# jinbeizame007/pytorch-r2d2-DPG

Hardware: NVIDIA H100
Metric: learner sequence-steps/sec (batch x seq_len) (higher is better)
Workload: dtype bf16x3 (fp32 operands split into bf16 hi+lo, three tensor-core passes, fp32 accumulate: ~16-bit operands)

## Files before the change

pytorch-r2d2-dpg_b200/csrc/learner.cu:

```cuda
#include "learner.cuh"

#include <cmath>
#include <stdlib.h>

#include "elementwise.cuh"
#include "gemm.cuh"
#include "lstm_scan.cuh"
#include "td3.cuh"

namespace r2d2 {

static size_t align64(size_t n) { return (n + 63) & ~(size_t)63; }

int learner_create(Learner** out, const r2d2_learner_config* cfg, bool twin_critic) {
  R2D2_REQUIRE(out && cfg, "null");
  R2D2_REQUIRE(cfg->obs_size > 0 && cfg->n_actions > 0 && cfg->hidden > 0 && cfg->hidden % 4 == 0, "sizes");
  R2D2_REQUIRE(cfg->batch > 0 && cfg->burn_in >= 0 && cfg->learning > 0 && cfg->n_step > 0, "window");
  R2D2_REQUIRE(cfg->learning >= 2, "learning >= 2: the [b:-1:B] priority series of the last batch element drops its "
                                   "last TD step, so a one-step window leaves it empty");
  R2D2_REQUIRE(cfg->actor_params && cfg->critic_params && cfg->target_actor_params && cfg->target_critic_params,
               "parameter buffers");
  R2D2_REQUIRE(cfg->actor_grads && cfg->critic_grads && cfg->actor_exp_avg && cfg->actor_exp_avg_sq &&
                   cfg->critic_exp_avg && cfg->critic_exp_avg_sq, "gradient / Adam buffers");
  Learner* l = new Learner();
  l->cfg = *cfg;
  l->actor_sh = NetShape{cfg->obs_size, cfg->n_actions, cfg->hidden, false};
  l->critic_sh = NetShape{cfg->obs_size, cfg->n_actions, cfg->hidden, true};
  const int B = cfg->batch, Bn = cfg->burn_in, L = cfg->learning, n = cfg->n_step;
  const int O = cfg->obs_size, A = cfg->n_actions, H = cfg->hidden;
  const int Tt = Bn + n + L, Tc = Bn + L, Tw = Bn + L + n;
  l->rows = Tw;
  size_t total = 0;
  const size_t n_obs = align64((size_t)Tw * B * O), n_act = align64((size_t)Tw * B * A), n_rt = align64((size_t)Tw * B);
  const size_t n_states = align64((size_t)8 * B * H), n_lba = align64((size_t)L * B * A);
  const size_t n_acttc = align64((size_t)Tt * B * A);
  total += 2 * (n_obs + n_act + 2 * n_rt + n_states + align64(B)  + align64(2 * (size_t)B) );
  total += n_acttc + 8 * n_lba + align64((size_t)L * B) + align64(B) + 64;
  const size_t ws_ta = ChainWs::floats(l->actor_sh, Tt, B, 1), ws_tc = ChainWs::floats(l->critic_sh, Tt, B, 1);
  const size_t ws_c1 = ChainWs::floats(l->critic_sh, Tc, B, 1), ws_a1 = ChainWs::floats(l->actor_sh, L, B, 2);
  const size_t ws_c2 = ChainWs::floats(l->critic_sh, L, B, 1);
  total += ws_ta + ws_tc + ws_c1 + ws_a1 + ws_c2;
  total += 2 * align64(B);
  total += align64(8) + align64(4 * (size_t)kGradNormBlocks);
  l->twin = twin_critic;
  if (twin_critic) {
    l->twin_floats = align64(ws_tc) + align64(ws_c1) + 3 * n_lba + align64((size_t)L * B);
    total += l->twin_floats;
  }
  R2D2_CUDA_TRY(cudaMalloc(&l->arena, total * sizeof(float)));
  R2D2_CUDA_TRY(cudaMemset(l->arena, 0, total * sizeof(float)));
  l->arena_floats = total;
  float* p = l->arena;
  auto take = [&](size_t nfl) { float* r = p; p += align64(nfl); return r; };
  for (auto& b : l->slots) {
    b.obs = take(n_obs); b.act = take(n_act); b.rew = take(n_rt); b.term = take(n_rt);
    b.states = take(n_states); b.uniforms = take(B);
    b.leaf_idx = reinterpret_cast<long long*>(take(2 * (size_t)B));
  }
  learner_select_batch(l, 0);
  l->act_tc = take(n_acttc);
  l->q = take(n_lba); l->q_next = take(n_lba); l->target = take(n_lba); l->dq = take(n_lba);
  l->mu = take(n_lba); l->q_pi = take(n_lba); l->dq_pi = take(n_lba); l->dpre_actor = take(n_lba);
  l->td_sq = take((size_t)L * B); l->priority = take(B); l->losses = take(64);
  l->ws_ta = ChainWs::carve(take(ws_ta), l->actor_sh, Tt, B, 1);
  l->ws_tc = ChainWs::carve(take(ws_tc), l->critic_sh, Tt, B, 1);
  l->ws_c1 = ChainWs::carve(take(ws_c1), l->critic_sh, Tc, B, 1);
  l->ws_a1 = ChainWs::carve(take(ws_a1), l->actor_sh, L, B, 2);
  l->ws_c2 = ChainWs::carve(take(ws_c2), l->critic_sh, L, B, 1);
  l->ws_ta.inference_only = true;
  l->ws_tc.inference_only = true;
  for (auto& b : l->slots) {
    b.is_weight = take(B);
    R2D2_TRY(fill_f32(b.is_weight, B, 1.0f, 0));
  }
  l->optim = take(8);
  l->norm_ticket = reinterpret_cast<unsigned int*>(l->optim + 4);
  l->norm_part = reinterpret_cast<double*>(take(4 * (size_t)kGradNormBlocks));
  if (twin_critic) {
    l->ws_tc_2 = ChainWs::carve(take(ws_tc), l->critic_sh, Tt, B, 1);
    l->ws_c1_2 = ChainWs::carve(take(ws_c1), l->critic_sh, Tc, B, 1);
    l->ws_tc_2.inference_only = true;
    l->q_next2 = take(n_lba); l->q2 = take(n_lba); l->dq2 = take(n_lba);
    l->td_sq2 = take((size_t)L * B);
  }
  R2D2_CUDA_TRY(cudaStreamSynchronize(0));
  learner_select_batch(l, 0);
  {
    const char* e = getenv("R2D2_OVERLAP_INPUTS");
    l->overlap_inputs = !(e && e[0] == '0');
    if (l->overlap_inputs) {
      int lo = 0, hi = 0;
      R2D2_CUDA_TRY(cudaDeviceGetStreamPriorityRange(&lo, &hi));
      R2D2_CUDA_TRY(cudaStreamCreateWithPriority(&l->side, cudaStreamNonBlocking, lo));
      R2D2_CUDA_TRY(cudaEventCreateWithFlags(&l->ev_fork, cudaEventDisableTiming));
      R2D2_CUDA_TRY(cudaEventCreateWithFlags(&l->ev_c1_inputs, cudaEventDisableTiming));
      R2D2_CUDA_TRY(cudaEventCreateWithFlags(&l->ev_a1_inputs, cudaEventDisableTiming));
    }
  }
  *out = l;
  return R2D2_OK;
}

int learner_destroy(Learner* l) {
  if (!l) return R2D2_OK;
  if (l->side) { cudaStreamSynchronize(l->side); cudaStreamDestroy(l->side); }
  if (l->ev_fork) cudaEventDestroy(l->ev_fork);
  if (l->ev_c1_inputs) cudaEventDestroy(l->ev_c1_inputs);
  if (l->ev_a1_inputs) cudaEventDestroy(l->ev_a1_inputs);
  cudaFree(l->arena);
  cudaFree(l->metrics_part);
  delete l->peer;
  delete l;
  return R2D2_OK;
}

int learner_select_batch(Learner* l, int slot) {
  R2D2_REQUIRE(l && (slot == 0 || slot == 1), "batch slot");
  const Learner::BatchSlot& b = l->slots[slot];
  l->cur_slot = slot;
  l->obs = b.obs; l->act = b.act; l->rew = b.rew; l->term = b.term; l->states = b.states; l->uniforms = b.uniforms;
  l->leaf_idx = b.leaf_idx; l->is_weight = b.is_weight;
  return R2D2_OK;
}

int learner_discard_prefetch(Learner* l, cudaStream_t st) {
  R2D2_REQUIRE(l, "null");
  if (l->c1_inputs_slot >= 0 && l->side) R2D2_CUDA_TRY(cudaStreamWaitEvent(st, l->ev_c1_inputs, 0));
  l->c1_inputs_slot = -1;
  l->targets_slot = -1;
  return R2D2_OK;
}

int learner_target_phase(Learner* l, int slot, cudaStream_t st) {
  R2D2_REQUIRE(l && (slot == 0 || slot == 1), "batch slot");
  const r2d2_learner_config& c = l->cfg;
  const int B = c.batch, Bn = c.burn_in, L = c.learning, n = c.n_step, A = c.n_actions, H = c.hidden;
  const int Tt = Bn + n + L, Tc = Bn + L;
  const long long launches0 = launch_count();
  const Learner::BatchSlot& b = l->slots[slot];
  const bool ahead = slot != l->cur_slot;
  const NetParams Pa_t = NetParams::from_flat(c.target_actor_params, l->actor_sh);
  const NetParams Pc_t = NetParams::from_flat(c.target_critic_params, l->critic_sh);
  const size_t BH = (size_t)B * H;
  const float* st_ta = b.states + 2 * BH;
  const float* st_tc = b.states + 6 * BH;

  R2D2_TRY(net_forward_inputs(l->actor_sh, Pa_t, l->ws_ta, b.obs, nullptr, Tt, B, st));
  if (l->overlap_inputs) {
    bool forked = false;
    auto fork = [&]() -> int {
      if (!forked) {
        R2D2_CUDA_TRY(cudaEventRecord(l->ev_fork, st));
        R2D2_CUDA_TRY(cudaStreamWaitEvent(l->side, l->ev_fork, 0));
        forked = true;
      }
      return R2D2_OK;
    };
    if (!ahead && l->c1_inputs_slot != slot) {
      const NetParams Pc = NetParams::from_flat(c.critic_params, l->critic_sh);
      R2D2_TRY(fork());
      R2D2_TRY(net_forward_inputs(l->critic_sh, Pc, l->ws_c1, b.obs, b.act, Tc, B, l->side));
      R2D2_CUDA_TRY(cudaEventRecord(l->ev_c1_inputs, l->side));
      l->c1_inputs_slot = slot;
    }
    if ((ahead || l->overlap_actor_inputs) && !l->a1_inputs_pending && !l->actor_forward_done) {
      const NetParams Pa = NetParams::from_flat(c.actor_params, l->actor_sh);
      R2D2_TRY(fork());
      R2D2_TRY(net_forward_inputs(l->actor_sh, Pa, l->ws_a1, l->obs + (size_t)Bn * B * c.obs_size, nullptr, L, B, l->side));
      R2D2_CUDA_TRY(cudaEventRecord(l->ev_a1_inputs, l->side));
      l->a1_inputs_pending = true;
    }
  }
  R2D2_TRY(net_forward_scan(l->actor_sh, Pa_t, l->ws_ta, st_ta, st_ta + BH, Tt, B, 1, st));
  if (l->peer) {
    R2D2_TRY(peer_reduce(*l->peer, kPeerCritic, st));
    R2D2_TRY(peer_reduce(*l->peer, kPeerActor, st));
  }
  R2D2_CUDA_TRY(cudaMemcpyAsync(l->act_tc, b.act, sizeof(float) * (size_t)(Bn + n) * B * A, cudaMemcpyDeviceToDevice, st));
  float* act_next = l->act_tc + (size_t)(Bn + n) * B * A;
  R2D2_TRY(net_head_forward(l->actor_sh, Pa_t, l->ws_ta, Bn + n, Tt, B, 1, act_next, A, st));
  if (l->target_noise > 0.0f)
    R2D2_TRY(target_smoothing(act_next, act_next, (long long)L * B * A, l->target_noise, l->target_noise_clip,
                              l->noise_seed, l->noise_rank, (unsigned long long)l->critic_iters, st));
  R2D2_TRY(net_forward(l->critic_sh, Pc_t, l->ws_tc, b.obs, l->act_tc, st_tc, st_tc + BH, Tt, B, 1, st));
  R2D2_TRY(net_head_forward(l->critic_sh, Pc_t, l->ws_tc, Bn + n, Tt, B, 1, l->q_next, A, st));
  if (l->twin) {
    const NetParams Pc_t2 = NetParams::from_flat(c.target_critic_params + l->critic_stride(), l->critic_sh);
    R2D2_TRY(net_forward(l->critic_sh, Pc_t2, l->ws_tc_2, b.obs, l->act_tc, nullptr, nullptr, Tt, B, 1, st));
    R2D2_TRY(net_head_forward(l->critic_sh, Pc_t2, l->ws_tc_2, Bn + n, Tt, B, 1, l->q_next2, A, st));
    R2D2_TRY(q_min(l->q_next, l->q_next2, (long long)L * B * A, st));
  }
  l->targets_slot = slot;
  l->launches_target = (int)(launch_count() - launches0);
  return R2D2_OK;
}

int learner_critic_phase(Learner* l, cudaStream_t st) {
  const r2d2_learner_config& c = l->cfg;
  const int B = c.batch, Bn = c.burn_in, L = c.learning, n = c.n_step, A = c.n_actions, H = c.hidden;
  const int Tc = Bn + L;
  const long long launches0 = launch_count();
  const NetParams Pc = NetParams::from_flat(c.critic_params, l->critic_sh);
  const NetParams Gc = NetParams::from_flat(c.critic_grads, l->critic_sh);
  const size_t BH = (size_t)B * H;
  const float* st_c = l->states + 4 * BH;

  l->target_phase_standalone = l->targets_slot == l->cur_slot;
  if (!l->target_phase_standalone) R2D2_TRY(learner_target_phase(l, l->cur_slot, st));
  if (l->c1_inputs_slot == l->cur_slot) R2D2_CUDA_TRY(cudaStreamWaitEvent(st, l->ev_c1_inputs, 0));
  else R2D2_TRY(net_forward_inputs(l->critic_sh, Pc, l->ws_c1, l->obs, l->act, Tc, B, st));
  l->c1_inputs_slot = -1;
  R2D2_TRY(net_forward_scan(l->critic_sh, Pc, l->ws_c1, st_c, st_c + BH, Tc, B, 1, st));
  if (l->peer) R2D2_TRY(peer_reduce(*l->peer, kPeerActor, st));
  R2D2_TRY(net_head_forward(l->critic_sh, Pc, l->ws_c1, Bn, Tc, B, 1, l->q, A, st));
  l->targets_slot = -1;

  TdPriorityParams tp;
  tp.q = l->q; tp.q_next = l->q_next; tp.rew = l->rew; tp.term = l->term;
  tp.target = l->target; tp.dq = l->dq; tp.td_sq = l->td_sq; tp.priority = l->priority; tp.loss_sum = l->losses;
  tp.L = L; tp.B = B; tp.A = A; tp.burn_in = Bn; tp.n_step = n;
  tp.gamma_n = (float)std::pow((double)c.gamma, (double)n);
  tp.eta = c.eta;
  tp.is_weight = l->importance_weighting ? l->is_weight : nullptr;
  R2D2_TRY(td_priority(tp, st, TdOptions{l->rescaling, l->rescaling_eps, l->priority_metric}));

  R2D2_CUDA_TRY(cudaMemsetAsync(c.critic_grads, 0, sizeof(float) * l->critic_block(), st));
  R2D2_TRY(net_backward(l->critic_sh, Pc, &Gc, l->ws_c1, l->obs, l->act, l->dq, Bn, Tc, B, 1, nullptr, nullptr, st));
  if (l->twin) {
    const size_t off = l->critic_stride();
    const NetParams Pc2 = NetParams::from_flat(c.critic_params + off, l->critic_sh);
    const NetParams Gc2 = NetParams::from_flat(c.critic_grads + off, l->critic_sh);
    R2D2_TRY(net_forward(l->critic_sh, Pc2, l->ws_c1_2, l->obs, l->act, nullptr, nullptr, Tc, B, 1, st));
    R2D2_TRY(net_head_forward(l->critic_sh, Pc2, l->ws_c1_2, Bn, Tc, B, 1, l->q2, A, st));
    TdPriorityParams tp2 = tp;
    tp2.q = l->q2; tp2.target = nullptr; tp2.dq = l->dq2; tp2.td_sq = l->td_sq2; tp2.priority = nullptr;
    tp2.loss_sum = l->losses + 2;
    R2D2_TRY(td_priority(tp2, st, TdOptions{l->rescaling, l->rescaling_eps, l->priority_metric}));
    R2D2_TRY(net_backward(l->critic_sh, Pc2, &Gc2, l->ws_c1_2, l->obs, l->act, l->dq2, Bn, Tc, B, 1, nullptr, nullptr,
                          st));
  }
  if (l->peer) R2D2_TRY(peer_signal(*l->peer, kPeerCritic, st));
  l->critic_phase_ran = true;
  l->metrics_iter = l->critic_iters;
  if (l->metrics_ring) {
    MetricsCriticParams mp;
    mp.q = l->q; mp.target = l->target; mp.q2 = l->twin ? l->q2 : nullptr; mp.priority = l->priority;
    mp.is_weight = l->importance_weighting ? l->is_weight : nullptr; mp.losses = l->losses;
    mp.n = (long long)L * B * A; mp.B = B; mp.iter = l->metrics_iter; mp.rec = l->metrics_record(l->metrics_iter);
    R2D2_TRY(metrics_critic(mp, l->metrics_part, l->metrics_ticket, st));
  }
  l->critic_iters += 1;
  l->launches_phase[0] = (int)(launch_count() - launches0);
  return R2D2_OK;
}

int learner_actor_forward(Learner* l, cudaStream_t st) {
  const r2d2_learner_config& c = l->cfg;
  const int B = c.batch, Bn = c.burn_in, L = c.learning, A = c.n_actions, O = c.obs_size;
  const long long launches0 = launch_count();
  const NetParams Pa = NetParams::from_flat(c.actor_params, l->actor_sh);
  const float* obs_l = l->obs + (size_t)Bn * B * O;
  if (l->a1_inputs_pending) {
    R2D2_CUDA_TRY(cudaStreamWaitEvent(st, l->ev_a1_inputs, 0));
    l->a1_inputs_pending = false;
  } else {
    R2D2_TRY(net_forward_inputs(l->actor_sh, Pa, l->ws_a1, obs_l, nullptr, L, B, st));
  }
  if (l->peer) R2D2_TRY(peer_reduce(*l->peer, kPeerCritic, st));
  R2D2_TRY(net_forward_scan(l->actor_sh, Pa, l->ws_a1, nullptr, nullptr, L, B, 2, st));
  R2D2_TRY(net_head_forward(l->actor_sh, Pa, l->ws_a1, 0, L, B, 2, l->mu, A, st));
  l->actor_forward_done = true;
  l->launches_actor_forward = (int)(launch_count() - launches0);
  return R2D2_OK;
}

static bool updates_targets(const Learner* l) {
  const int k = l->cfg.target_update_interval;
  return k > 0 && (l->step + 1) % k == 0;
}

static int optimiser_step(Learner* l, int block, float* params, float* exp_avg, float* exp_avg_sq, float* target,
                          long long n, float lr, float grad_scale, cudaStream_t st) {
  const float* grads = l->optimiser_grads(block);
  const float* coef = nullptr;
  if (l->grad_clip > 0.0f || l->metrics_ring) {
    R2D2_TRY(grad_norm(grads, n, grad_scale, l->grad_clip, l->norm_part + (size_t)block * kGradNormBlocks,
                       l->norm_ticket + block, l->optim + block, l->optim + 2 + block, st));
    if (l->grad_clip > 0.0f) coef = l->optim + 2 + block;
  }
  const bool polyak = l->target_tau < 1.0f && updates_targets(l);
  return adam_step(params, grads, exp_avg, exp_avg_sq, n, l->step + 1, lr, 0.9f, 0.999f, 1e-8f, grad_scale, st, coef,
                   polyak ? target : nullptr, l->target_tau);
}

int learner_actor_phase(Learner* l, float grad_scale, cudaStream_t st) {
  const r2d2_learner_config& c = l->cfg;
  const int B = c.batch, Bn = c.burn_in, L = c.learning, A = c.n_actions, O = c.obs_size;
  const long long launches0 = launch_count();
  const NetParams Pa = NetParams::from_flat(c.actor_params, l->actor_sh);
  const NetParams Ga = NetParams::from_flat(c.actor_grads, l->actor_sh);
  const NetParams Pc = NetParams::from_flat(c.critic_params, l->critic_sh);
  const long long LBA = (long long)L * B * A;

  int extra = 0;
  if (!l->actor_forward_done) R2D2_TRY(learner_actor_forward(l, st));
  else extra = l->launches_actor_forward;
  l->actor_forward_done = false;
  const long long launches1 = launch_count();
  (void)launches1;
  if (l->peer) R2D2_TRY(peer_wait(*l->peer, kPeerCritic, st));
  R2D2_TRY(optimiser_step(l, kPeerCritic, c.critic_params, c.critic_exp_avg, c.critic_exp_avg_sq, c.target_critic_params,
                          (long long)l->critic_block(), c.critic_lr, grad_scale, st));
  {
    const int other = 1 - l->cur_slot;
    if (l->overlap_inputs && l->targets_slot == other && l->c1_inputs_slot != other) {
      const Learner::BatchSlot& nb = l->slots[other];
      R2D2_CUDA_TRY(cudaEventRecord(l->ev_fork, st));
      R2D2_CUDA_TRY(cudaStreamWaitEvent(l->side, l->ev_fork, 0));
      R2D2_TRY(net_forward_inputs(l->critic_sh, Pc, l->ws_c1, nb.obs, nb.act, Bn + L, B, l->side));
      R2D2_CUDA_TRY(cudaEventRecord(l->ev_c1_inputs, l->side));
      l->c1_inputs_slot = other;
    }
  }

  const float* obs_l = l->obs + (size_t)Bn * B * O;
  R2D2_TRY(net_forward(l->critic_sh, Pc, l->ws_c2, obs_l, l->mu, nullptr, nullptr, L, B, 1, st));
  R2D2_TRY(net_head_forward(l->critic_sh, Pc, l->ws_c2, 0, L, B, 1, l->q_pi, A, st));
  R2D2_TRY(scaled_sum(l->q_pi, LBA, -1.0f / (float)LBA, l->losses + 1, st));
  if (l->metrics_ring) {
    MetricsActorParams mp;
    mp.mu = l->mu; mp.losses = l->losses; mp.critic_norm = l->optim + kPeerCritic; mp.n = LBA;
    mp.rec = l->metrics_record(l->metrics_iter);
    R2D2_TRY(metrics_actor(mp, l->metrics_part, l->metrics_ticket, st));
  }
  R2D2_TRY(fill_f32(l->dq_pi, LBA, -1.0f / (float)LBA, st));
  R2D2_TRY(net_backward(l->critic_sh, Pc, nullptr, l->ws_c2, obs_l, l->mu, l->dq_pi, 0, L, B, 1, l->dpre_actor,
                        l->mu, st));
  R2D2_CUDA_TRY(cudaMemsetAsync(c.actor_grads, 0, sizeof(float) * l->actor_sh.param_count(), st));
  R2D2_TRY(net_backward(l->actor_sh, Pa, &Ga, l->ws_a1, obs_l, nullptr, l->dpre_actor, 0, L, B, 2, nullptr, nullptr, st));
  if (l->peer) R2D2_TRY(peer_signal(*l->peer, kPeerActor, st));
  l->launches_phase[1] = (int)(launch_count() - launches0) + extra;
  return R2D2_OK;
}

int learner_finish_phase(Learner* l, float grad_scale, cudaStream_t st) {
  const r2d2_learner_config& c = l->cfg;
  const long long launches0 = launch_count();
  if (l->peer) R2D2_TRY(peer_wait(*l->peer, kPeerActor, st));
  R2D2_TRY(optimiser_step(l, kPeerActor, c.actor_params, c.actor_exp_avg, c.actor_exp_avg_sq, c.target_actor_params,
                          (long long)l->actor_sh.param_count(), c.actor_lr, grad_scale, st));
  if (l->metrics_ring)
    R2D2_CUDA_TRY(cudaMemcpyAsync(l->metrics_actor_norms() + l->step % l->metrics_slots, l->optim + kPeerActor,
                                  sizeof(float), cudaMemcpyDeviceToDevice, st));
  l->step += 1;
  if (l->target_tau == 1.0f && c.target_update_interval > 0 && l->step % c.target_update_interval == 0) {
    R2D2_CUDA_TRY(cudaMemcpyAsync(c.target_actor_params, c.actor_params, sizeof(float) * l->actor_sh.param_count(),
                                  cudaMemcpyDeviceToDevice, st));
    R2D2_CUDA_TRY(cudaMemcpyAsync(c.target_critic_params, c.critic_params, sizeof(float) * l->critic_block(),
                                  cudaMemcpyDeviceToDevice, st));
  }
  l->launches_phase[2] = (int)(launch_count() - launches0);
  return R2D2_OK;
}

int learner_set_metrics(Learner* l, void* ring, int slots) {
  R2D2_REQUIRE(l, "null");
  R2D2_REQUIRE(!ring || slots >= 1, "slots >= 1");
  R2D2_REQUIRE(((uintptr_t)ring & 7) == 0, "the ring holds doubles: 8-byte aligned");
  if (l->critic_phase_ran) {
    set_last_error("metrics are switched on or off before the first critic phase");
    return R2D2_ERR_STATE;
  }
  if (ring && !l->metrics_part) {
    const size_t n = (size_t)kMetricsBlocks * kMetricsPartials;
    R2D2_CUDA_TRY(cudaMalloc(&l->metrics_part, n * sizeof(double) + 64));
    R2D2_CUDA_TRY(cudaMemset(l->metrics_part, 0, n * sizeof(double) + 64));
    R2D2_CUDA_TRY(cudaDeviceSynchronize());
    l->metrics_ticket = reinterpret_cast<unsigned int*>(l->metrics_part + n);
  }
  l->metrics_ring = static_cast<double*>(ring);
  l->metrics_slots = ring ? slots : 0;
  return R2D2_OK;
}

int learner_attach_peers(Learner* l, int rank, int world, void* const* peer_bases) {
  R2D2_REQUIRE(l && peer_bases, "null argument");
  R2D2_REQUIRE(world >= 2 && world <= kPeerMaxWorld && rank >= 0 && rank < world, "peer rank / world");
  R2D2_REQUIRE(!l->peer, "peers already attached");
  PeerExchange* x = new PeerExchange();
  x->rank = rank;
  x->world = world;
  x->lay = peer_layout((long long)l->critic_block(), (long long)l->actor_sh.param_count(), world);
  for (int k = 0; k < world; ++k) {
    if (!peer_bases[k]) { delete x; R2D2_REQUIRE(false, "null peer buffer"); }
    x->ptrs.base[k] = static_cast<char*>(peer_bases[k]);
  }
  l->peer = x;
  l->cfg.critic_grads = x->grads(kPeerCritic);
  l->cfg.actor_grads = x->grads(kPeerActor);
  return R2D2_OK;
}

}
```

pytorch-r2d2-dpg_b200/csrc/learner.cuh:

```cuda
#pragma once
#include "common.cuh"
#include "elementwise.cuh"
#include "metrics.cuh"
#include "net.cuh"
#include "peer.cuh"

namespace r2d2 {

struct Learner {
  r2d2_learner_config cfg;
  NetShape actor_sh, critic_sh;
  int rows = 0;
  int step = 0;
  int launches_phase[3] = {0, 0, 0};
  cudaStream_t side = nullptr;
  cudaEvent_t ev_fork = nullptr, ev_c1_inputs = nullptr, ev_a1_inputs = nullptr;
  bool overlap_inputs = false;
  bool overlap_actor_inputs = true;
  bool a1_inputs_pending = false;
  bool actor_forward_done = false;
  int launches_actor_forward = 0;
  float* arena = nullptr;
  size_t arena_floats = 0;
  struct BatchSlot {
    float *obs = nullptr, *act = nullptr, *rew = nullptr, *term = nullptr, *states = nullptr, *uniforms = nullptr;
    long long* leaf_idx = nullptr;
    float* is_weight = nullptr;
  } slots[2];
  int cur_slot = 0;
  int targets_slot = -1;
  int c1_inputs_slot = -1;
  int launches_target = 0;
  bool target_phase_standalone = false;
  float *obs = nullptr, *act = nullptr, *rew = nullptr, *term = nullptr, *states = nullptr, *uniforms = nullptr;
  long long* leaf_idx = nullptr;
  float* is_weight = nullptr;
  bool importance_weighting = false;
  float target_tau = 1.0f;
  float grad_clip = 0.0f;
  float* optim = nullptr;
  unsigned int* norm_ticket = nullptr;
  double* norm_part = nullptr;
  int rescaling = kRescaleReference;
  float rescaling_eps = 0.0f;
  int priority_metric = kPrioritySquared;
  bool twin = false;
  float target_noise = 0.0f, target_noise_clip = 0.5f;
  unsigned int noise_seed = 0, noise_rank = 0;
  long long critic_iters = 0;
  size_t twin_floats = 0;
  size_t critic_stride() const { return twin ? (critic_sh.param_count() + 63) & ~(size_t)63 : critic_sh.param_count(); }
  size_t critic_block() const { return critic_stride() * (twin ? 2 : 1); }
  float *act_tc = nullptr, *q = nullptr, *q_next = nullptr, *target = nullptr, *dq = nullptr, *mu = nullptr,
        *q_pi = nullptr, *dq_pi = nullptr, *dpre_actor = nullptr, *td_sq = nullptr, *priority = nullptr,
        *losses = nullptr;
  ChainWs ws_ta, ws_tc, ws_c1, ws_a1, ws_c2;
  ChainWs ws_tc_2, ws_c1_2;
  float *q_next2 = nullptr, *q2 = nullptr, *dq2 = nullptr, *td_sq2 = nullptr;
  PeerExchange* peer = nullptr;
  double* metrics_ring = nullptr;
  int metrics_slots = 0;
  double* metrics_part = nullptr;
  unsigned int* metrics_ticket = nullptr;
  long long metrics_iter = 0;
  bool critic_phase_ran = false;
  double* metrics_record(long long iter) const { return metrics_ring + (size_t)(iter % metrics_slots) * kMetricsFields; }
  float* metrics_actor_norms() const {
    return reinterpret_cast<float*>(metrics_ring + (size_t)metrics_slots * kMetricsFields);
  }
  const float* optimiser_grads(int block) const {
    return peer ? peer->sums(block) : (block == kPeerCritic ? cfg.critic_grads : cfg.actor_grads);
  }
};

int learner_create(Learner** out, const r2d2_learner_config* cfg, bool twin_critic = false);
int learner_destroy(Learner* l);
int learner_select_batch(Learner* l, int slot);
int learner_target_phase(Learner* l, int slot, cudaStream_t stream);
int learner_discard_prefetch(Learner* l, cudaStream_t stream);
int learner_critic_phase(Learner* l, cudaStream_t stream);
int learner_actor_forward(Learner* l, cudaStream_t stream);
int learner_actor_phase(Learner* l, float grad_scale, cudaStream_t stream);
int learner_finish_phase(Learner* l, float grad_scale, cudaStream_t stream);
int learner_attach_peers(Learner* l, int rank, int world, void* const* peer_bases);
int learner_set_metrics(Learner* l, void* ring, int slots);

}
```

Before: 1.158 million.

## Run actor forward and critic backward on an auxiliary stream concurrently

Adds a second low-priority side stream and uses it for two things: launching the actor forward at the start of the critic phase, and running the critic backward pass, the twin-critic forward/backward and the metrics on it, all forked from the main stream with events. The aim is to let independent LSTM chains use the GPU at the same time instead of running one after another. New events keep q_next from being overwritten before the twin TD reads it, and make the actor phase wait for the auxiliary work to finish. This adds event overhead and contention between streams, and leaves more cross-iteration ordering hazards to get right.

```diff
diff --git a/pytorch-r2d2-dpg_b200/csrc/learner.cu b/pytorch-r2d2-dpg_b200/csrc/learner.cu
--- a/pytorch-r2d2-dpg_b200/csrc/learner.cu
+++ b/pytorch-r2d2-dpg_b200/csrc/learner.cu
@@ -92,9 +92,10 @@
       int lo = 0, hi = 0;
       R2D2_CUDA_TRY(cudaDeviceGetStreamPriorityRange(&lo, &hi));
       R2D2_CUDA_TRY(cudaStreamCreateWithPriority(&l->side, cudaStreamNonBlocking, lo));
-      R2D2_CUDA_TRY(cudaEventCreateWithFlags(&l->ev_fork, cudaEventDisableTiming));
-      R2D2_CUDA_TRY(cudaEventCreateWithFlags(&l->ev_c1_inputs, cudaEventDisableTiming));
-      R2D2_CUDA_TRY(cudaEventCreateWithFlags(&l->ev_a1_inputs, cudaEventDisableTiming));
+      R2D2_CUDA_TRY(cudaStreamCreateWithPriority(&l->aux, cudaStreamNonBlocking, lo));
+      for (cudaEvent_t* ev : {&l->ev_fork, &l->ev_c1_inputs, &l->ev_a1_inputs, &l->ev_aux_fork, &l->ev_aux_done,
+                              &l->ev_q_next_read})
+        R2D2_CUDA_TRY(cudaEventCreateWithFlags(ev, cudaEventDisableTiming));
     }
   }
   *out = l;
@@ -104,9 +105,9 @@
 int learner_destroy(Learner* l) {
   if (!l) return R2D2_OK;
   if (l->side) { cudaStreamSynchronize(l->side); cudaStreamDestroy(l->side); }
-  if (l->ev_fork) cudaEventDestroy(l->ev_fork);
-  if (l->ev_c1_inputs) cudaEventDestroy(l->ev_c1_inputs);
-  if (l->ev_a1_inputs) cudaEventDestroy(l->ev_a1_inputs);
+  if (l->aux) { cudaStreamSynchronize(l->aux); cudaStreamDestroy(l->aux); }
+  for (cudaEvent_t ev : {l->ev_fork, l->ev_c1_inputs, l->ev_a1_inputs, l->ev_aux_fork, l->ev_aux_done, l->ev_q_next_read})
+    if (ev) cudaEventDestroy(ev);
   cudaFree(l->arena);
   cudaFree(l->metrics_part);
   delete l->peer;
@@ -126,6 +127,7 @@
 int learner_discard_prefetch(Learner* l, cudaStream_t st) {
   R2D2_REQUIRE(l, "null");
   if (l->c1_inputs_slot >= 0 && l->side) R2D2_CUDA_TRY(cudaStreamWaitEvent(st, l->ev_c1_inputs, 0));
+  if (l->aux_pending) R2D2_CUDA_TRY(cudaStreamWaitEvent(st, l->ev_aux_done, 0));
   l->c1_inputs_slot = -1;
   l->targets_slot = -1;
   return R2D2_OK;
@@ -183,6 +185,10 @@
     R2D2_TRY(target_smoothing(act_next, act_next, (long long)L * B * A, l->target_noise, l->target_noise_clip,
                               l->noise_seed, l->noise_rank, (unsigned long long)l->critic_iters, st));
   R2D2_TRY(net_forward(l->critic_sh, Pc_t, l->ws_tc, b.obs, l->act_tc, st_tc, st_tc + BH, Tt, B, 1, st));
+  if (l->q_next_pending) {
+    R2D2_CUDA_TRY(cudaStreamWaitEvent(st, l->ev_q_next_read, 0));
+    l->q_next_pending = false;
+  }
   R2D2_TRY(net_head_forward(l->critic_sh, Pc_t, l->ws_tc, Bn + n, Tt, B, 1, l->q_next, A, st));
   if (l->twin) {
     const NetParams Pc_t2 = NetParams::from_flat(c.target_critic_params + l->critic_stride(), l->critic_sh);
@@ -204,7 +210,19 @@
   const NetParams Gc = NetParams::from_flat(c.critic_grads, l->critic_sh);
   const size_t BH = (size_t)B * H;
   const float* st_c = l->states + 4 * BH;
-
+  const bool concurrent = l->concurrent_chains();
+  auto fork_aux = [&]() -> int {
+    R2D2_CUDA_TRY(cudaEventRecord(l->ev_aux_fork, st));
+    R2D2_CUDA_TRY(cudaStreamWaitEvent(l->aux, l->ev_aux_fork, 0));
+    return R2D2_OK;
+  };
+
+  int actor_launches = 0;
+  if (concurrent && !l->actor_forward_done) {
+    R2D2_TRY(fork_aux());
+    R2D2_TRY(learner_actor_forward(l, l->aux));
+    actor_launches = l->launches_actor_forward;
+  }
   l->target_phase_standalone = l->targets_slot == l->cur_slot;
   if (!l->target_phase_standalone) R2D2_TRY(learner_target_phase(l, l->cur_slot, st));
   if (l->c1_inputs_slot == l->cur_slot) R2D2_CUDA_TRY(cudaStreamWaitEvent(st, l->ev_c1_inputs, 0));
@@ -224,20 +242,29 @@
   tp.is_weight = l->importance_weighting ? l->is_weight : nullptr;
   R2D2_TRY(td_priority(tp, st, TdOptions{l->rescaling, l->rescaling_eps, l->priority_metric}));
 
-  R2D2_CUDA_TRY(cudaMemsetAsync(c.critic_grads, 0, sizeof(float) * l->critic_block(), st));
-  R2D2_TRY(net_backward(l->critic_sh, Pc, &Gc, l->ws_c1, l->obs, l->act, l->dq, Bn, Tc, B, 1, nullptr, nullptr, st));
+  cudaStream_t bs = st;
+  if (concurrent) {
+    R2D2_TRY(fork_aux());
+    bs = l->aux;
+  }
+  R2D2_CUDA_TRY(cudaMemsetAsync(c.critic_grads, 0, sizeof(float) * l->critic_block(), bs));
+  R2D2_TRY(net_backward(l->critic_sh, Pc, &Gc, l->ws_c1, l->obs, l->act, l->dq, Bn, Tc, B, 1, nullptr, nullptr, bs));
   if (l->twin) {
     const size_t off = l->critic_stride();
     const NetParams Pc2 = NetParams::from_flat(c.critic_params + off, l->critic_sh);
     const NetParams Gc2 = NetParams::from_flat(c.critic_grads + off, l->critic_sh);
-    R2D2_TRY(net_forward(l->critic_sh, Pc2, l->ws_c1_2, l->obs, l->act, nullptr, nullptr, Tc, B, 1, st));
-    R2D2_TRY(net_head_forward(l->critic_sh, Pc2, l->ws_c1_2, Bn, Tc, B, 1, l->q2, A, st));
+    R2D2_TRY(net_forward(l->critic_sh, Pc2, l->ws_c1_2, l->obs, l->act, nullptr, nullptr, Tc, B, 1, bs));
+    R2D2_TRY(net_head_forward(l->critic_sh, Pc2, l->ws_c1_2, Bn, Tc, B, 1, l->q2, A, bs));
     TdPriorityParams tp2 = tp;
     tp2.q = l->q2; tp2.target = nullptr; tp2.dq = l->dq2; tp2.td_sq = l->td_sq2; tp2.priority = nullptr;
     tp2.loss_sum = l->losses + 2;
-    R2D2_TRY(td_priority(tp2, st, TdOptions{l->rescaling, l->rescaling_eps, l->priority_metric}));
+    R2D2_TRY(td_priority(tp2, bs, TdOptions{l->rescaling, l->rescaling_eps, l->priority_metric}));
+    if (concurrent) {
+      R2D2_CUDA_TRY(cudaEventRecord(l->ev_q_next_read, bs));
+      l->q_next_pending = true;
+    }
     R2D2_TRY(net_backward(l->critic_sh, Pc2, &Gc2, l->ws_c1_2, l->obs, l->act, l->dq2, Bn, Tc, B, 1, nullptr, nullptr,
-                          st));
+                          bs));
   }
   if (l->peer) R2D2_TRY(peer_signal(*l->peer, kPeerCritic, st));
   l->critic_phase_ran = true;
@@ -247,14 +274,19 @@
     mp.q = l->q; mp.target = l->target; mp.q2 = l->twin ? l->q2 : nullptr; mp.priority = l->priority;
     mp.is_weight = l->importance_weighting ? l->is_weight : nullptr; mp.losses = l->losses;
     mp.n = (long long)L * B * A; mp.B = B; mp.iter = l->metrics_iter; mp.rec = l->metrics_record(l->metrics_iter);
-    R2D2_TRY(metrics_critic(mp, l->metrics_part, l->metrics_ticket, st));
+    R2D2_TRY(metrics_critic(mp, l->metrics_part, l->metrics_ticket, bs));
+  }
+  if (concurrent) {
+    R2D2_CUDA_TRY(cudaEventRecord(l->ev_aux_done, l->aux));
+    l->aux_pending = true;
   }
   l->critic_iters += 1;
-  l->launches_phase[0] = (int)(launch_count() - launches0);
+  l->launches_phase[0] = (int)(launch_count() - launches0) - actor_launches;
   return R2D2_OK;
 }
 
 int learner_actor_forward(Learner* l, cudaStream_t st) {
+  if (l->actor_forward_done) return R2D2_OK;
   const r2d2_learner_config& c = l->cfg;
   const int B = c.batch, Bn = c.burn_in, L = c.learning, A = c.n_actions, O = c.obs_size;
   const long long launches0 = launch_count();
@@ -302,6 +334,10 @@
   const NetParams Pc = NetParams::from_flat(c.critic_params, l->critic_sh);
   const long long LBA = (long long)L * B * A;
 
+  if (l->aux_pending) {
+    R2D2_CUDA_TRY(cudaStreamWaitEvent(st, l->ev_aux_done, 0));
+    l->aux_pending = false;
+  }
   int extra = 0;
   if (!l->actor_forward_done) R2D2_TRY(learner_actor_forward(l, st));
   else extra = l->launches_actor_forward;
diff --git a/pytorch-r2d2-dpg_b200/csrc/learner.cuh b/pytorch-r2d2-dpg_b200/csrc/learner.cuh
--- a/pytorch-r2d2-dpg_b200/csrc/learner.cuh
+++ b/pytorch-r2d2-dpg_b200/csrc/learner.cuh
@@ -20,6 +20,11 @@
   bool a1_inputs_pending = false;
   bool actor_forward_done = false;
   int launches_actor_forward = 0;
+  cudaStream_t aux = nullptr;
+  cudaEvent_t ev_aux_fork = nullptr, ev_aux_done = nullptr, ev_q_next_read = nullptr;
+  bool aux_pending = false;
+  bool q_next_pending = false;
+  bool concurrent_chains() const { return aux && overlap_actor_inputs && !peer; }
   float* arena = nullptr;
   size_t arena_floats = 0;
   struct BatchSlot {
```

Measured after the change: 1.241 million (median of 6 runs). 7.2% higher.
